# LLaVA-VL/LLaVA-Plus-Codebase

Measured on NVIDIA H100. Metric: prefill+decode tokens/s, higher is better.
Workload: dtype bf16

## Files before the change

### llava-plus-codebase_b200/csrc/decode_mega.cu

```cuda
#include <limits.h>
#include <math.h>

#include "common.cuh"
#include "kernels.h"

namespace b2 {
namespace {

constexpr int MK_CONS_WARPS = 16;
constexpr int MK_CONS = MK_CONS_WARPS * 32;
constexpr int MK_PROD_WARPS = 4;
constexpr int MK_THREADS = MK_CONS + 32 * MK_PROD_WARPS;
constexpr int MK_D = 128;
constexpr int MK_U = 4;
constexpr int MK_KT = 2048;
constexpr int MK_ROW_PAD = 64;
constexpr int MK_ROW_STRIDE = MK_KT * 2 + MK_ROW_PAD;
constexpr int MK_TILE_BYTES = 8 * MK_ROW_STRIDE;
constexpr int MK_MAXNB = 32;
constexpr int MK_MAXL = 48;
constexpr int MK_MAX_STAGES = 12;

__device__ __forceinline__ void unpack8(const uint4& u, float (&f)[8]) {
    f[0] = bf16_lo(u.x); f[1] = bf16_hi(u.x); f[2] = bf16_lo(u.y); f[3] = bf16_hi(u.y);
    f[4] = bf16_lo(u.z); f[5] = bf16_hi(u.z); f[6] = bf16_lo(u.w); f[7] = bf16_hi(u.w);
}
__device__ __forceinline__ uint4 ldcg16(const void* p) { return __ldcg(reinterpret_cast<const uint4*>(p)); }

__device__ __forceinline__ void cons_sync() { asm volatile("bar.sync 1, %0;" ::"n"(MK_CONS) : "memory"); }

__device__ __forceinline__ void grid_sync(unsigned int* counter, unsigned int target) {
    cons_sync();
    if (threadIdx.x == 0) {
        asm volatile("red.release.gpu.global.add.u32 [%0], 1;" ::"l"(counter) : "memory");
        unsigned int cur, spins = 0;
        do {
            asm volatile("ld.acquire.gpu.global.u32 %0, [%1];" : "=r"(cur) : "l"(counter) : "memory");
            if (++spins > (1u << 26)) asm volatile("trap;");
        } while ((int)(cur - target) < 0);
    }
    cons_sync();
}

__device__ __forceinline__ void bulk_g2s(void* smem_dst, const void* gsrc, uint32_t bytes, uint64_t* bar) {
    asm volatile("cp.async.bulk.shared::cluster.global.mbarrier::complete_tx::bytes [%0], [%1], %2, [%3];" ::"r"(
                     smem_u32(smem_dst)),
                 "l"(gsrc), "r"(bytes), "r"(smem_u32(bar))
                 : "memory");
}

struct GemvCtx {
    const __nv_bfloat16* W;
    int K, act;
    int u_lo, nu;
    int nb;
    int nchunk;
};
struct PhaseIO {
    const __nv_bfloat16* xin;
    const __nv_bfloat16* gamma;
    const __nv_bfloat16* residual;
    void* out;
    int ld_out, out_fp32;
};

__device__ __forceinline__ int mk_phys_row(const GemvCtx& c, int rb, int g, bool& valid) {
    if (c.act == ACT_SWIGLU) {
        const int lc = rb * 4 + (g & 3);
        valid = lc < c.nu;
        const int ch = c.u_lo + lc;
        return (ch >> 6) * 128 + (ch & 63) + ((g >> 2) ? 64 : 0);
    }
    const int lr = rb * 8 + g;
    valid = lr < c.nu;
    return c.u_lo + lr;
}

__device__ __forceinline__ int mk_rows_in_block(const GemvCtx& c, int rb) {
    if (c.act == ACT_SWIGLU) return 2 * min(4, c.nu - rb * 4);
    return min(8, c.nu - rb * 8);
// ... 79 lines not shown
#pragma unroll
                for (int e = 0; e < 8; ++e) o[e] = gf[e] * round_bf16(f[e] * rstd);
                *px = make_uint4(pack_bf16(o[0], o[1]), pack_bf16(o[2], o[3]), pack_bf16(o[4], o[5]),
                                 pack_bf16(o[6], o[7]));
            }
        }
    }
    cons_sync();
}

__device__ __forceinline__ void mk_mma(float (&c)[4], uint32_t a0, uint32_t a2, uint32_t b0, uint32_t b1) {
    asm volatile(
        "mma.sync.aligned.m16n8k16.row.col.f32.bf16.bf16.f32 {%0,%1,%2,%3}, {%4,%5,%6,%7}, {%8,%9}, {%0,%1,%2,%3};"
        : "+f"(c[0]), "+f"(c[1]), "+f"(c[2]), "+f"(c[3])
        : "r"(a0), "r"(0u), "r"(a2), "r"(0u), "r"(b0), "r"(b1));
}

template <int NB>
__device__ __forceinline__ float mk_row_value(const float* s_gpart, int rb, int b, int r) {
    float v = 0.f;
#pragma unroll
    for (int ww = 0; ww < MK_CONS_WARPS; ++ww) v += s_gpart[(((size_t)ww * MK_MAXNB + rb) * NB + b) * 8 + r];
    return v;
}

template <int NB>
__device__ __forceinline__ void mk_epilogue(const MegaParams& p, const MegaLayer* layers, int ph, const GemvCtx& c,
                                            int B, int tid, const float* s_gpart, float res_pref, bool have_res_pref) {
    const PhaseIO io = mk_phase_io(p, layers, ph);
    if (c.act == ACT_SWIGLU) {
        const int nch = c.nu;
        for (int idx = tid; idx < nch * B; idx += MK_CONS) {
            const int b = idx / nch, r = idx - b * nch;
            const int rb = r >> 2, q = r & 3;
            const float gt = mk_row_value<NB>(s_gpart, rb, b, q);
            const float up = mk_row_value<NB>(s_gpart, rb, b, q + 4);
            reinterpret_cast<__nv_bfloat16*>(io.out)[(size_t)b * io.ld_out + (size_t)c.u_lo + r] =
                __float2bfloat16_rn(gt / (1.0f + __expf(-gt)) * up);
        }
    } else {
        const int nr = c.nu;
        for (int idx = tid; idx < nr * B; idx += MK_CONS) {
            const int b = idx / nr, r = idx - b * nr;
            float y = mk_row_value<NB>(s_gpart, r >> 3, b, r & 7);
            const size_t o = (size_t)b * io.ld_out + (size_t)c.u_lo + r;
            if (io.residual != nullptr) y += have_res_pref ? res_pref : __bfloat162float(__ldcg(io.residual + o));
            if (io.out_fp32) reinterpret_cast<float*>(io.out)[o] = y;
            else reinterpret_cast<__nv_bfloat16*>(io.out)[o] = __float2bfloat16_rn(y);
        }
    }
}

__device__ __forceinline__ void mk_attention(const MegaParams& p, const MegaLayer& Lw, int tid, int lane, int warp,
                                             float (*s_part)[MK_D + 2], int* s_flag, const float* s_cos,
                                             const float* s_sin) {
    const int h = p.h, H = p.H;
    const int pairs = p.B * H;
    const int grid = gridDim.x;
    const int G = pairs <= grid ? grid / pairs : 1;
    const int hw = lane >> 4, c = lane & 15;
    const int split = pairs <= grid ? (int)blockIdx.x % G : 0;
    for (int pair = pairs <= grid ? (int)blockIdx.x / G : (int)blockIdx.x; pair < pairs;
         pair += (pairs <= grid ? pairs : grid)) {
        const int head = pair % H, b = pair / H;
        const int pos = p.cur_len[b];
        const int total = pos + 1;
        const int cchunk = (total + G - 1) / G;
        const int cb = split * cchunk;
        const int ce = min(cb + cchunk, total);
        const int wchunk = (max(ce - cb, 0) + MK_CONS_WARPS - 1) / MK_CONS_WARPS;
        const int k_begin = cb + warp * wchunk;
        const int k_end = min(k_begin + wchunk, ce);
        const __nv_bfloat16* qrow = p.qkv + (size_t)b * 3 * h + head * MK_D;
        float qreg[8], knew[8], vnew[8];
        {
            float qa[8], qb[8], ka[8], kb[8];
            unpack8(ldcg16(qrow + c * 8), qa);
            unpack8(ldcg16(qrow + (c ^ 8) * 8), qb);
            unpack8(ldcg16(qrow + h + c * 8), ka);
            unpack8(ldcg16(qrow + h + (c ^ 8) * 8), kb);
            unpack8(ldcg16(qrow + 2 * h + c * 8), vnew);
            const float sign = (c < 8) ? -1.f : 1.f;
#pragma unroll
            for (int e = 0; e < 8; ++e) {
                const int i = ((c & 7) * 8 + e);
                const float cbf = s_cos[b * 64 + i], sbf = s_sin[b * 64 + i];
                qreg[e] = round_bf16(round_bf16(qa[e] * cbf) + round_bf16(sign * qb[e] * sbf));
                knew[e] = round_bf16(round_bf16(ka[e] * cbf) + round_bf16(sign * kb[e] * sbf));
            }
        }
        const size_t cbase = ((size_t)b * H + head) * p.Smax * MK_D;
        if (pos >= k_begin && pos < k_end && hw == 0) {
            *reinterpret_cast<uint4*>(Lw.kcache + cbase + (size_t)pos * MK_D + c * 8) =
                make_uint4(pack_bf16(knew[0], knew[1]), pack_bf16(knew[2], knew[3]),
                           pack_bf16(knew[4], knew[5]), pack_bf16(knew[6], knew[7]));
            *reinterpret_cast<uint4*>(Lw.vcache + cbase + (size_t)pos * MK_D + c * 8) =
                make_uint4(pack_bf16(vnew[0], vnew[1]), pack_bf16(vnew[2], vnew[3]),
                           pack_bf16(vnew[4], vnew[5]), pack_bf16(vnew[6], vnew[7]));
        }
        float m_run = -INFINITY, l_run = 0.f, av[8];
#pragma unroll
        for (int e = 0; e < 8; ++e) av[e] = 0.f;
        const __nv_bfloat16* kb_ = Lw.kcache + cbase + c * 8;
        const __nv_bfloat16* vb_ = Lw.vcache + cbase + c * 8;
        for (int kbase = k_begin; kbase < k_end; kbase += 2 * MK_U) {
            uint4 kraw[MK_U], vraw[MK_U];
#pragma unroll
// ... 26 lines not shown
                dot += __shfl_xor_sync(0xffffffffu, dot, 1);
                if (key < k_end) {
                    const float sc = dot * p.scale_log2;
                    const float m_new = fmaxf(m_run, sc);
                    const float corr = exp2f(m_run - m_new);
                    const float pr = exp2f(sc - m_new);
                    l_run = l_run * corr + pr;
#pragma unroll
                    for (int e = 0; e < 8; ++e) av[e] = av[e] * corr + pr * vf[e];
                    m_run = m_new;
                }
            }
        }
        {
            const float m_o = __shfl_xor_sync(0xffffffffu, m_run, 16);
            const float l_o = __shfl_xor_sync(0xffffffffu, l_run, 16);
            const float m_c = fmaxf(m_run, m_o);
            const float w_s = (m_run == -INFINITY) ? 0.f : exp2f(m_run - m_c);
            const float w_o = (m_o == -INFINITY) ? 0.f : exp2f(m_o - m_c);
#pragma unroll
            for (int e = 0; e < 8; ++e) {
                const float a_o = __shfl_xor_sync(0xffffffffu, av[e], 16);
                av[e] = av[e] * w_s + a_o * w_o;
            }
            l_run = l_run * w_s + l_o * w_o;
            m_run = m_c;
        }
        if (hw == 0) {
#pragma unroll
            for (int e = 0; e < 8; ++e) s_part[warp][c * 8 + e] = av[e];
            if (c == 0) { s_part[warp][MK_D] = m_run; s_part[warp][MK_D + 1] = l_run; }
        }
        cons_sync();
        float m_cta = -INFINITY, l_cta = 0.f, o_cta = 0.f;
        if (tid < MK_D) {
#pragma unroll
            for (int i = 0; i < MK_CONS_WARPS; ++i) m_cta = fmaxf(m_cta, s_part[i][MK_D]);
#pragma unroll
            for (int i = 0; i < MK_CONS_WARPS; ++i) {
                const float ms = s_part[i][MK_D];
                const float wgt = (ms == -INFINITY) ? 0.f : exp2f(ms - m_cta);
                l_cta += s_part[i][MK_D + 1] * wgt;
                o_cta += s_part[i][tid] * wgt;
            }
        }
        if (G == 1) {
            if (tid < MK_D) p.attn[(size_t)b * h + head * MK_D + tid] = __float2bfloat16_rn(o_cta / l_cta);
        } else {
            float* part = p.attn_partial + ((size_t)pair * G + split) * (MK_D + 2);
            if (tid < MK_D) {
                part[tid] = o_cta;
                if (tid == 0) { part[MK_D] = m_cta; part[MK_D + 1] = l_cta; }
            }
            __threadfence();
            cons_sync();
            if (tid == 0) *s_flag = (atomicAdd(&p.attn_counters[pair], 1) == G - 1) ? 1 : 0;
            cons_sync();
            if (*s_flag) {
                __threadfence();
                if (tid < MK_D) {
                    const float* pb = p.attn_partial + (size_t)pair * G * (MK_D + 2);
                    float m_all = -INFINITY;
                    for (int sidx = 0; sidx < G; ++sidx) m_all = fmaxf(m_all, __ldcg(pb + (size_t)sidx * (MK_D + 2) + MK_D));
                    float l_all = 0.f, o_all = 0.f;
                    for (int sidx = 0; sidx < G; ++sidx) {
                        const float ms = __ldcg(pb + (size_t)sidx * (MK_D + 2) + MK_D);
                        const float wgt = (ms == -INFINITY) ? 0.f : exp2f(ms - m_all);
                        l_all += __ldcg(pb + (size_t)sidx * (MK_D + 2) + MK_D + 1) * wgt;
                        o_all += __ldcg(pb + (size_t)sidx * (MK_D + 2) + tid) * wgt;
                    }
                    p.attn[(size_t)b * h + head * MK_D + tid] = __float2bfloat16_rn(o_all / l_all);
                    if (tid == 0) p.attn_counters[pair] = 0;
                }
            }
        }
        cons_sync();
    }
}

struct TileCursor {
    GemvCtx c;
    int ph, rb, kc;
    uint32_t tile;
    bool valid;
};
__device__ __forceinline__ void cursor_seek(TileCursor& t, const MegaParams& p, const MegaLayer* layers, int n_phases) {
    while (t.ph < n_phases) {
        if (!mk_is_attention(p, t.ph)) {
            t.c = mk_phase_ctx(p, layers, t.ph);
            if (t.c.nb > 0) { t.rb = 0; t.kc = 0; t.valid = true; return; }
        }
        ++t.ph;
    }
    t.valid = false;
}
__device__ __forceinline__ void cursor_begin(TileCursor& t, const MegaParams& p, const MegaLayer* layers, int n_phases) {
    t.ph = 0; t.tile = 0; t.rb = 0; t.kc = 0;
    cursor_seek(t, p, layers, n_phases);
}
__device__ __forceinline__ void cursor_next(TileCursor& t, const MegaParams& p, const MegaLayer* layers, int n_phases) {
    ++t.tile;
    if (++t.kc < t.c.nchunk) return;
    t.kc = 0;
    if (++t.rb < t.c.nb) return;
    ++t.ph;
    cursor_seek(t, p, layers, n_phases);
}
template <int NB>
__global__ void __launch_bounds__(MK_THREADS, 1) decode_mega_kernel(MegaParams p, int n_stages) {
    extern __shared__ __align__(128) uint8_t mk_smem[];
    uint8_t* ring = mk_smem;
    __nv_bfloat16* xs = reinterpret_cast<__nv_bfloat16*>(ring + (size_t)n_stages * MK_TILE_BYTES);
    float* s_gpart = reinterpret_cast<float*>(reinterpret_cast<uint8_t*>(xs) + (size_t)NB * (p.h > p.I ? p.h : p.I) * 2);
    uint64_t* full_bar = reinterpret_cast<uint64_t*>(s_gpart + (size_t)MK_CONS_WARPS * MK_MAXNB * NB * 8);
    uint64_t* empty_bar = full_bar + MK_MAX_STAGES;
    __shared__ float s_red[MK_CONS_WARPS][NB];
    __shared__ float s_rstd[NB];
    __shared__ float s_av[MK_CONS_WARPS];
    __shared__ int s_ai[MK_CONS_WARPS];
    __shared__ float s_part[MK_CONS_WARPS][MK_D + 2];
    __shared__ int s_flag;
    __shared__ float s_cos[NB * 64], s_sin[NB * 64];
    __shared__ __align__(16) MegaLayer s_layers[MK_MAXL];

    const int tid = threadIdx.x, lane = tid & 31, warp = tid >> 5;
    const int B = p.B;
    const int n_phases = 5 * p.L + 1;

    {
        const uint4* src = reinterpret_cast<const uint4*>(p.layers);
        uint4* dst = reinterpret_cast<uint4*>(s_layers);
        for (int i = tid; i < p.L * (int)(sizeof(MegaLayer) / 16); i += MK_THREADS) dst[i] = src[i];
        if (tid == 0) {
            for (int s = 0; s < n_stages; ++s) {
                mbar_init(&full_bar[s], 1);
                mbar_init(&empty_bar[s], MK_CONS_WARPS);
            }
            fence_barrier_init();
        }
        __syncthreads();
    }

    if (warp >= MK_CONS_WARPS) {
        const uint32_t pw = (uint32_t)(warp - MK_CONS_WARPS);
        TileCursor cp;
        cursor_begin(cp, p, s_layers, n_phases);
        while (cp.valid) {
            if (cp.tile % (uint32_t)MK_PROD_WARPS == pw) {
                const uint32_t stage = cp.tile % (uint32_t)n_stages;
                const uint32_t parity = (cp.tile / (uint32_t)n_stages) & 1u;
                const uint32_t row_bytes = (uint32_t)min(MK_KT, cp.c.K - cp.kc * MK_KT) * 2u;
                if (lane == 0) {
                    mbar_wait(&empty_bar[stage], parity ^ 1u);
                    mbar_arrive_expect_tx(&full_bar[stage], (uint32_t)mk_rows_in_block(cp.c, cp.rb) * row_bytes);
                }
                __syncwarp();
                bool row_valid;
                const int prow = mk_phys_row(cp.c, cp.rb, lane & 7, row_valid);
                if (lane < 8 && row_valid)
                    bulk_g2s(ring + (size_t)stage * MK_TILE_BYTES + (size_t)lane * MK_ROW_STRIDE,
                             cp.c.W + (size_t)prow * cp.c.K + (size_t)cp.kc * MK_KT, row_bytes, &full_bar[stage]);
            }
            cursor_next(cp, p, s_layers, n_phases);
        }
        return;
    }

    for (int i = tid; i < B * 64; i += MK_CONS) {
        const int b = i >> 6, f = i & 63;
        const float inv_freq = exp2f(-(2.0f * f / MK_D) * log2f(p.theta));
        float sv, cv;
        sincosf((float)p.cur_len[b] * inv_freq, &sv, &cv);
        s_cos[i] = round_bf16(cv);
        s_sin[i] = round_bf16(sv);
    }
    if (blockIdx.x < B) {
        int t = p.tok[blockIdx.x];
        t = t < 0 ? 0 : (t >= p.V ? p.V - 1 : t);
        const uint4* src = reinterpret_cast<const uint4*>(p.embed + (size_t)t * p.h);
        uint4* dst = reinterpret_cast<uint4*>(p.x + (size_t)blockIdx.x * p.h);
        for (int i = tid; i < p.h / 8; i += MK_CONS) dst[i] = src[i];
    }
    __nv_bfloat16* gsm = xs + (size_t)NB * p.h;
    const bool gsm_fits = (size_t)(NB + 1) * p.h <= (size_t)NB * (p.h > p.I ? p.h : p.I);
    auto gamma_prefetch = [&](int ph) -> bool {
        if (!gsm_fits || ph >= n_phases || mk_is_attention(p, ph)) return false;
        const PhaseIO io = mk_phase_io(p, s_layers, ph);
        if (io.gamma == nullptr) return false;
        for (int i = tid; i < (p.h >> 3); i += MK_CONS)
            asm volatile("cp.async.cg.shared.global [%0], [%1], 16;" ::"r"(smem_u32(gsm + i * 8)), "l"(io.gamma + i * 8) : "memory");
        asm volatile("cp.async.commit_group;" ::: "memory");
        return true;
    };
    bool gsm_ok = gamma_prefetch(0);
    unsigned int bar_target = p.bar_base + gridDim.x;
    grid_sync(p.bar_count, bar_target);

    const bool tracing = p.trace != nullptr && blockIdx.x == 0 && tid == 0;
    const int g = lane >> 2, t4 = lane & 3;
    uint32_t tile = 0;
#pragma unroll 1
    for (int ph = 0; ph < n_phases; ++ph) {
        if (tracing) p.trace[ph * 4 + 0] = clock64();
        if (mk_is_attention(p, ph)) {
            mk_attention(p, s_layers[ph / 5], tid, lane, warp, s_part, &s_flag, s_cos, s_sin);
        } else {
            const GemvCtx c = mk_phase_ctx(p, s_layers, ph);
            const PhaseIO io = mk_phase_io(p, s_layers, ph);
            const bool have_res = io.residual != nullptr && c.nu * B <= MK_CONS;
            float res_pref = 0.f;
            if (have_res && tid < c.nu * B) {
                const int b = tid / c.nu, r = tid - b * c.nu;
                res_pref = __bfloat162float(__ldcg(io.residual + (size_t)b * io.ld_out + (size_t)c.u_lo + r));
            }
            mk_prologue<NB>(io, c.K, B, p.eps, tid, lane, warp, xs, s_red, s_rstd, gsm_ok ? gsm : nullptr);
            if (tracing) p.trace[ph * 4 + 1] = clock64();
#pragma unroll 1
            for (int rb = 0; rb < c.nb; ++rb) {
                float acc[4] = {0.f, 0.f, 0.f, 0.f}, acc2[4] = {0.f, 0.f, 0.f, 0.f};
#pragma unroll 1
                for (int kc = 0; kc < c.nchunk; ++kc, ++tile) {
                    const uint32_t stage = tile % (uint32_t)n_stages;
                    const uint32_t parity = (tile / (uint32_t)n_stages) & 1u;
                    const int nk32 = min(MK_KT, c.K - kc * MK_KT) >> 5;
                    mbar_wait(&full_bar[stage], parity);
                    const uint8_t* trow = ring + (size_t)stage * MK_TILE_BYTES + (size_t)g * MK_ROW_STRIDE + t4 * 16;
                    const __nv_bfloat16* xrow = xs + (size_t)g * c.K + (size_t)kc * MK_KT + t4 * 8;
#pragma unroll 4
                    for (int k32 = warp; k32 < nk32; k32 += MK_CONS_WARPS) {
                        const uint4 wv = *reinterpret_cast<const uint4*>(trow + k32 * 64);
                        uint4 xv = make_uint4(0, 0, 0, 0);
                        if (g < B) xv = *reinterpret_cast<const uint4*>(xrow + k32 * 32);
                        mk_mma(acc, xv.x, xv.y, wv.x, wv.y);
                        mk_mma(acc2, xv.z, xv.w, wv.z, wv.w);
                    }
                    __syncwarp();
                    if (lane == 0) mbar_arrive(&empty_bar[stage]);
                }
                if (g < NB)
                    *reinterpret_cast<float2*>(s_gpart + (((size_t)warp * MK_MAXNB + rb) * NB + g) * 8 + t4 * 2) =
                        make_float2(acc[0] + acc2[0], acc[1] + acc2[1]);
            }
            cons_sync();
            if (tracing) p.trace[ph * 4 + 2] = clock64();
            mk_epilogue<NB>(p, s_layers, ph, c, B, tid, s_gpart, res_pref, have_res);
        }
        if (tracing) p.trace[ph * 4 + 3] = clock64();
        gsm_ok = gamma_prefetch(ph + 1);
        bar_target += gridDim.x;
        grid_sync(p.bar_count, bar_target);
    }
    if (tracing) p.trace[n_phases * 4] = clock64();

    if (blockIdx.x < B) {
        const int b = blockIdx.x;
        const float* row = p.logits + (size_t)b * p.V;
        float best = -INFINITY;
        int bi = INT_MAX;
        for (int i = tid; i < p.V; i += MK_CONS) {
            const float v = __ldcg(row + i);
            if (v == v && (bi == INT_MAX || v > best)) { best = v; bi = i; }
        }
#pragma unroll
        for (int o = 16; o > 0; o >>= 1) {
            const float ov = __shfl_xor_sync(0xffffffffu, best, o);
            const int oi = __shfl_xor_sync(0xffffffffu, bi, o);
            if (ov > best || (ov == best && oi < bi)) { best = ov; bi = oi; }
        }
        if (lane == 0) { s_av[warp] = best; s_ai[warp] = bi; }
        cons_sync();
        if (warp == 0) {
            best = lane < MK_CONS_WARPS ? s_av[lane] : -INFINITY;
            bi = lane < MK_CONS_WARPS ? s_ai[lane] : INT_MAX;
#pragma unroll
            for (int o = 16; o > 0; o >>= 1) {
                const float ov = __shfl_xor_sync(0xffffffffu, best, o);
                const int oi = __shfl_xor_sync(0xffffffffu, bi, o);
                if (ov > best || (ov == best && oi < bi)) { best = ov; bi = oi; }
            }
            if (lane == 0) {
                const int tk = bi == INT_MAX ? 0 : bi;
                p.tok[b] = tk;
                p.out_tokens[(size_t)(*p.step_counter) * B + b] = tk;
                if (p.rows == nullptr || p.rows[b].active) p.cur_len[b] += 1;
                if (p.ring != nullptr) {
                    const int pub = p.sstate->pub_counter, tag0 = p.sstate->tag;
                    if (tag0 != 0) {
                        const int tag = 1 + (tag0 - 1 + pub / p.ring_cap) % 2047;
                        reinterpret_cast<volatile int32_t*>(p.ring)[(size_t)(pub % p.ring_cap) * B + b] = (tag << 20) | (tk & 0xFFFFF);
                        __threadfence_system();
                    }
                }
            }
        }
    }
    cons_sync();
    if (tid == 0) {
        __threadfence();
        if (atomicAdd(p.done_count, 1u) == gridDim.x - 1) {
            *p.done_count = 0u;
            *p.step_counter += 1;
            if (p.ring != nullptr) p.sstate->pub_counter += 1;
        }
    }
}

size_t mega_fixed_bytes(int NB, int h, int I) {
    return (size_t)NB * (h > I ? h : I) * 2 + (size_t)MK_CONS_WARPS * MK_MAXNB * NB * 8 * 4 + 2 * MK_MAX_STAGES * 8;
}
size_t mega_static_bytes(int NB) {
    return (size_t)(MK_CONS_WARPS + 1) * NB * 4 + MK_CONS_WARPS * (MK_D + 2 + 2) * 4 + NB * 512 +
           MK_MAXL * sizeof(MegaLayer) + 1024;
}
int mega_stages(int NB, int h, int I) {
    const long long avail = 227 * 1024 - (long long)mega_fixed_bytes(NB, h, I) - (long long)mega_static_bytes(NB);
    long long s = avail / MK_TILE_BYTES;
    return (int)(s > MK_MAX_STAGES ? MK_MAX_STAGES : s);
}

}

bool decode_mega_fits(int B, int h, int I) {
    if (B < 1 || B > 2) return false;
    return mega_stages(B, h, I) >= 4;
}

int decode_mega(const MegaParams& p, cudaStream_t stream) {
    B2_CHECK_ARG(p.B >= 1 && p.B <= 2, "decode_mega: batch must be 1..2");
    B2_CHECK_ARG(p.L <= MK_MAXL, "decode_mega: %d layers exceed the shared layer table (%d)", p.L, MK_MAXL);
    B2_CHECK_ARG(p.h % 256 == 0 && p.I % 256 == 0 && p.V % 8 == 0 && p.h / p.H == MK_D,
                 "decode_mega: unsupported dims h=%d I=%d V=%d H=%d", p.h, p.I, p.V, p.H);
    {
        const int grid = num_sms();
        const int nmax = p.V > 3 * p.h ? (p.V > 2 * p.I ? p.V : 2 * p.I) : (3 * p.h > 2 * p.I ? 3 * p.h : 2 * p.I);
        B2_CHECK_ARG((nmax / 8 + grid - 1) / grid + 1 <= MK_MAXNB,
                     "decode_mega: %d output rows per CTA exceed the shared-memory block table", nmax / grid);
    }
    const int NB = p.B;
    const int stages = mega_stages(NB, p.h, p.I);
    B2_CHECK_ARG(stages >= 4, "decode_mega: shared memory too small for the weight ring (B=%d h=%d I=%d)", p.B, p.h, p.I);
    const size_t smem = (size_t)stages * MK_TILE_BYTES + mega_fixed_bytes(NB, p.h, p.I);
    void* fn = NB == 1 ? (void*)decode_mega_kernel<1> : (void*)decode_mega_kernel<2>;
    static size_t attr_smem[3] = {0, 0, 0};
    if (smem > attr_smem[NB]) {
        B2_CUDA_CHECK(cudaFuncSetAttribute(fn, cudaFuncAttributeMaxDynamicSharedMemorySize, (int)smem));
        attr_smem[NB] = smem;
    }
    MegaParams pp = p;
    int n_stages = stages;
    void* args[] = {&pp, &n_stages};
    B2_CUDA_CHECK(cudaLaunchCooperativeKernel(fn, dim3(num_sms()), dim3(MK_THREADS), args, smem, stream));
    B2_LAUNCH_CHECK();
    return 0;
}

}
```

### llava-plus-codebase_b200/csrc/kernels.h

```cpp
#pragma once
#include <cuda_bf16.h>
#include <cuda_runtime.h>
#include <stdint.h>

namespace b2 {

enum { ACT_NONE = 0, ACT_QUICK_GELU = 1, ACT_GELU_ERF = 2, ACT_SWIGLU = 3, ACT_ROPE_QKV = 4 };

struct RopeQkv {
    const void* table = nullptr;
    void* kcache = nullptr;
    void* vcache = nullptr;
    int S = 0, H = 0, Smax = 0;
    const int32_t* pos0 = nullptr;
};
enum { DT_BF16 = 0, DT_F16 = 1, DT_F32 = 2 };

int num_sms();

struct GemmArgs {
    const void* A = nullptr; int lda = 0;
    const void* W = nullptr; int ldw = 0;
    const void* bias = nullptr;
    const void* residual = nullptr; int ld_res = 0;
// ... 77 lines not shown
};
int flash_attn_bf16(const FlashArgs& a, cudaStream_t stream);

int rope_table_build(void* table, int Smax, int D, float theta, cudaStream_t stream);
int rope_kv_write(void* qkv, void* kcache, void* vcache, int B, int S, int H, int D, int Smax, float theta,
                  cudaStream_t stream, const int32_t* pos0 = nullptr);

struct DecodeAttnArgs {
    const void* qkv = nullptr;
    void* kcache = nullptr; void* vcache = nullptr;
    float* kscale = nullptr; float* vscale = nullptr;
    const int32_t* cur_len = nullptr;
    void* out = nullptr;
    float* partial = nullptr;
    int32_t* counters = nullptr;
    int B = 0, H = 0, D = 128, Smax = 0, nsplit = 1;
    float theta = 10000.f, scale = 1.f;
    int R = 1;
};
int decode_attn_ctas_per_sm();
int decode_attn_bf16(const DecodeAttnArgs& a, cudaStream_t stream);
int decode_attn_mq_ctas_per_sm();
size_t decode_attn_mq_scratch_bytes(int B, int H, int nsplit);
int decode_attn_mq_bf16(const DecodeAttnArgs& a, cudaStream_t stream);
constexpr int kPrefixGroupRows = 16;
struct PrefixGroup {
    int32_t src_slot, prefix_len, n_rows;
    int32_t rows[kPrefixGroupRows];
};
int decode_attn_shared_ctas_per_sm();
size_t decode_attn_shared_scratch_bytes(int B, int H, int nsplit);
int decode_attn_shared_bf16(const DecodeAttnArgs& a, const PrefixGroup* groups, const int32_t* row_prefix, int G,
                            cudaStream_t stream);
int decode_attn_e4m3_ctas_per_sm();
int decode_attn_e4m3(const DecodeAttnArgs& a, cudaStream_t stream);
int kv_quantize_e4m3(const void* ksrc, const void* vsrc, void* k8, void* v8, float* kscale, float* vscale,
                     const int32_t* seq_lens, int B, int S, int H, int D, int Smax, cudaStream_t stream,
                     const int32_t* pos0 = nullptr, int S_src = 0);
int kv_dequantize_e4m3(const void* k8, const void* v8, const float* kscale, const float* vscale, const int32_t* pos0, void* kdst,
                       void* vdst, int B, int H, int Smax, int S_dst, cudaStream_t stream);

struct MegaLayer {
    const __nv_bfloat16 *ln1, *wqkv, *wo, *ln2, *wgu, *wd;
    __nv_bfloat16 *kcache, *vcache;
};
struct MegaParams {
    const MegaLayer* layers = nullptr;
    int L = 0, h = 0, I = 0, H = 0, V = 0, B = 0, Smax = 0, nsplit = 1;
    const __nv_bfloat16 *embed = nullptr, *final_norm = nullptr, *lm_head = nullptr;
    int32_t *tok = nullptr, *cur_len = nullptr, *out_tokens = nullptr, *step_counter = nullptr;
    __nv_bfloat16 *x = nullptr, *qkv = nullptr, *attn = nullptr, *act = nullptr;
    float* logits = nullptr;
    float* attn_partial = nullptr;
    int32_t* attn_counters = nullptr;
    unsigned int *bar_count = nullptr, *done_count = nullptr;
    unsigned int bar_base = 0;
    float eps = 1e-5f, theta = 10000.f, scale_log2 = 1.f;
    long long* trace = nullptr;
    struct SampleState* sstate = nullptr;
    int32_t* ring = nullptr;
    int ring_cap = 0;
    const struct RowState* rows = nullptr;
};
int decode_mega(const MegaParams& p, cudaStream_t stream);
bool decode_mega_fits(int B, int h, int I);

struct SampleState {
    int do_sample;
    float temperature, top_p;
    int top_k;
    unsigned long long seed;
    int tag;
    int pub_counter;
    unsigned int done;
    int per_row;
    float* out_scores;
    float* out_logits;
    int out_cap;
};
struct RowState {
    int active;
    int do_sample; float temperature, top_p; int top_k;
    unsigned long long seed;
    int index;
};
constexpr int kProcMaxEos = 8;
struct ProcRow {
    int on;
    float penalty;
    int ngram;
    int min_gen;
    int n_eos;
    int eos[kProcMaxEos];
    int prompt_len;
    int hist_len;
};
struct ProcState {
    ProcRow* rows;
    int32_t* hist;
    uint32_t* bits;
    int cap, words;
};
constexpr int kSpecMaxRows = 16;
struct SpecState {
    int K;
    int ngram;
    int max_new;
    int n_eos;
    int eos[kProcMaxEos];
// ... 86 lines not shown
```

### llava-plus-codebase_b200/csrc/model.cu

```cuda
#include <cuda_fp16.h>
#include <limits.h>
#include <stdarg.h>
#include <stdio.h>
#include <stdlib.h>
#include <string.h>
#include <time.h>

#include <array>
#include <atomic>
#include <utility>
#include <mutex>
#include <string>
#include <vector>

#include "../../include/b2llava.h"
#include "common.cuh"
#include "kernels.h"

namespace b2 {

static thread_local char g_err[1024] = {0};
unsigned long long g_launch_count = 0;

void set_error(const char* fmt, ...) {
// ... 58 lines not shown
}

using namespace b2;

struct b2_model {
    b2_model_desc d;
    int device = 0;
    std::mutex mu;
    bool finalized = false;
    int P = 0, T = 0, kpad = 0, vit_live = 0, vit_hd = 64, hd = 128;
    DevBuf patch_w, cls, pos, pre_g, pre_b;
    std::vector<VitLayer> vit;
    DevBuf p0_w, p0_b, p2_w, p2_b;
    DevBuf embed, final_norm;
    Linear head;
    std::vector<LlamaLayer> ll;
    int* err_host = nullptr;
    int* err_dev = nullptr;
    cudaEvent_t ws_event = nullptr;
    cudaStream_t ws_stream = nullptr;
    bool ws_valid = false;
    DevBuf v_col, v_patch, v_hidden, v_xn, v_qkv, v_attn, v_mlp, v_feats, p_mid, p_done;
    DevBuf x, xn, qkv, attn, act, last_idx, xlast, logits, splice_idx;
    DevBuf chunk_pos;
    DevBuf enc_pixels, enc_out;
    std::vector<cudaGraphExec_t> enc_graph;
    std::vector<char> enc_warm;
    cudaStream_t enc_stream = nullptr;
    cudaEvent_t enc_fork = nullptr, enc_join = nullptr;
    int enc_launches = 0;
    bool fp8_decode = false;
    DevBuf xq8, xscale;
    DevBuf kstage, vstage;
    bool nf4 = false;
    DevBuf nf4_scratch;
    std::atomic<int> kv_live{0};
};

struct b2_kv {
    b2_model* m = nullptr;
    int max_batch = 0, max_seq = 0;
    int dtype = B2_KV_BF16;
    int pitch = 0;
    DevBuf k, v;
    DevBuf kscale, vscale;
    DevBuf len_dev, tok, step_counter, out_tokens, attn_partial, attn_counters;
    DevBuf sk_partial, sk_counters;
    std::vector<int32_t> len_host;
    int out_capacity = 0;
    cudaGraphExec_t graph = nullptr;
    int graph_B = 0;
    int graph_launches = 0;
    unsigned int mega_bar_base = 0;
    DevBuf mega_layers, mega_sync;
    DevBuf rope_tab;
    cudaStream_t own_stream = nullptr;
    cudaEvent_t ev_fork = nullptr, ev_join = nullptr;
    int warm_B = 0;
    DevBuf sstate;
    SampleState samp_host = {};
    bool samp_valid = false;
    int32_t* ring_host = nullptr;
    int32_t* ring_dev = nullptr;
    int ring_cap = 0;
    int epoch = 0;
    int stream_B = 0, stream_tag = 0, stream_scheduled = 0;
    float* next_scores = nullptr;
    float* next_logits = nullptr;
    int next_cap = 0;
    DevBuf rows_dev;
    std::vector<RowState> rows_host;
    DevBuf beam_in, beam_ws, beam_out;
    DevBuf proc_rows, proc_hist, proc_bits;
    std::vector<char> proc_on;
    bool any_proc() const { for (char c : proc_on) if (c) return true; return false; }
    DevBuf beam_proc_rows;
    bool beam_proc_on = false;
    DevBuf spec_state, spec_logits, spec_attn;
    int* spec_mirror = nullptr;
    int spec_nsplit = 0;
    int spec_R = 0;
    int spec_max_new = 0;
    int spec_queued = 0;
    int spec_len0 = 0;
    std::array<cudaGraphExec_t, kSpecMaxRows + 1> spec_graph{};
    std::array<int, kSpecMaxRows + 1> spec_launches{};
    std::array<char, kSpecMaxRows + 1> spec_warm{};
    DevBuf share_tab, share_attn;
    int share_G = 0;
    bool counted = false;
    bool e4m3() const { return dtype == B2_KV_E4M3; }
    size_t elem_bytes() const { return e4m3() ? 1 : 2; }
    size_t layer_rows() const { return (size_t)max_batch * m->d.heads * pitch; }
    size_t layer_stride() const { return layer_rows() * m->hd; }
    char* k_layer(int l) const { return k.as<char>() + (size_t)l * layer_stride() * elem_bytes(); }
    char* v_layer(int l) const { return v.as<char>() + (size_t)l * layer_stride() * elem_bytes(); }
};

namespace {

ProcState proc_state(const b2_kv* kv) {
    ProcState p = {};
    if (kv->proc_rows.p == nullptr) return p;
    p.rows = kv->proc_rows.as<ProcRow>(); p.hist = kv->proc_hist.as<int32_t>(); p.bits = kv->proc_bits.as<uint32_t>();
    p.cap = kv->max_seq + 1; p.words = (kv->m->d.vocab + 31) / 32;
    return p;
// ... 411 lines not shown
        B2_TRY(decode_linear(m, kv, p, L.d, lw.wd, m->act.p, I, nullptr, true, m->x.p, h, 0, B, h, I, ACT_NONE, st));
    }
    B2_TRY(decode_linear(m, kv, plan.head, m->head, m->head.w.p, m->x.p, h, m->final_norm.p, false, m->logits.p, V, 1, B, V, h,
                         ACT_NONE, st));
    B2_TRY(sample_publish(m->logits.as<float>(), V, B, kv->sstate.as<SampleState>(), kv->rows_dev.as<RowState>(), kv->tok.as<int32_t>(),
                          kv->out_tokens.as<int32_t>(), kv->step_counter.as<int32_t>(), kv->len_dev.as<int32_t>(),
                          kv->ring_dev, kv->ring_cap, SP_SELECT | SP_WRITE_OUT | SP_BUMP, 0, proc_state(kv), nullptr, st));
    return 0;
}

int fork_stream(b2_kv* kv, cudaStream_t st, cudaStream_t* run) {
    if (st != nullptr && st != cudaStreamLegacy) { *run = st; return 0; }
    if (kv->own_stream == nullptr) {
        B2_CUDA_CHECK(cudaStreamCreateWithFlags(&kv->own_stream, cudaStreamNonBlocking));
        B2_CUDA_CHECK(cudaEventCreateWithFlags(&kv->ev_fork, cudaEventDisableTiming));
        B2_CUDA_CHECK(cudaEventCreateWithFlags(&kv->ev_join, cudaEventDisableTiming));
    }
    B2_CUDA_CHECK(cudaEventRecord(kv->ev_fork, st));
    B2_CUDA_CHECK(cudaStreamWaitEvent(kv->own_stream, kv->ev_fork, 0));
    *run = kv->own_stream;
    return 0;
}
int join_stream(b2_kv* kv, cudaStream_t st, cudaStream_t run) {
    if (run == st) return 0;
    B2_CUDA_CHECK(cudaEventRecord(kv->ev_join, run));
    B2_CUDA_CHECK(cudaStreamWaitEvent(st, kv->ev_join, 0));
    return 0;
}

bool use_mega(const b2_model* m, const b2_kv* kv, int B) {
    if (kv->e4m3()) return false;
    if (m->nf4) return false;
    if (!decode_mega_fits(B, m->d.hidden, m->d.inter) || m->d.layers > 48) return false;
    static int flag = -1;
    if (flag < 0) {
        const char* e = getenv("B2_DECODE_MEGA");
        flag = (e != nullptr && e[0] == '0') ? 0 : 1;
    }
    return flag == 1;
}

int decode_step_mega(b2_model* m, b2_kv* kv, int B, cudaStream_t st) {
    const b2_model_desc& d = m->d;
    MegaParams p;
    p.layers = kv->mega_layers.as<MegaLayer>();
    p.L = d.layers; p.h = d.hidden; p.I = d.inter; p.H = d.heads; p.V = d.vocab; p.B = B; p.Smax = kv->pitch;
    int ns = (num_sms() * 16) / (B * d.heads);
    p.nsplit = ns < 1 ? 1 : (ns > 64 ? 64 : ns);
    p.embed = m->embed.as<bf16>(); p.final_norm = m->final_norm.as<bf16>(); p.lm_head = m->head.w.as<bf16>();
    p.tok = kv->tok.as<int32_t>(); p.cur_len = kv->len_dev.as<int32_t>();
    p.out_tokens = kv->out_tokens.as<int32_t>(); p.step_counter = kv->step_counter.as<int32_t>();
    p.x = m->x.as<bf16>(); p.qkv = m->qkv.as<bf16>(); p.attn = m->attn.as<bf16>(); p.act = m->act.as<bf16>();
    p.logits = m->logits.as<float>();
    p.attn_partial = kv->attn_partial.as<float>(); p.attn_counters = kv->attn_counters.as<int32_t>();
    unsigned int* sync = kv->mega_sync.as<unsigned int>();
    p.bar_count = sync; p.done_count = sync + 2;
    p.bar_base = kv->mega_bar_base;
    kv->mega_bar_base += (unsigned int)(5 * d.layers + 2) * (unsigned int)num_sms();
    p.eps = d.rms_eps; p.theta = d.rope_theta;
    p.scale_log2 = (1.0f / sqrtf((float)m->hd)) * 1.4426950408889634f;
    const bool sampling = kv->samp_host.do_sample != 0 || kv->samp_host.per_row != 0 || kv->any_proc();
    if (!sampling && kv->samp_host.tag != 0) { p.sstate = kv->sstate.as<SampleState>(); p.ring = kv->ring_dev; p.ring_cap = kv->ring_cap; }
    if (kv->samp_host.per_row) p.rows = kv->rows_dev.as<RowState>();
    static int trace_mode = -1;
    if (trace_mode < 0) { const char* e = getenv("B2_MEGA_TRACE"); trace_mode = (e && e[0] != 0) ? 1 : 0; }
    if (trace_mode == 1) {
        static int steps_seen = 0;
        if (++steps_seen == 40) {
            const int n = (5 * d.layers + 2) * 4;
            DevBuf tb;
            B2_TRY(tb.alloc((size_t)n * 8));
            cudaMemset(tb.p, 0, (size_t)n * 8);
            p.trace = tb.as<long long>();
            int r = decode_mega(p, st);
            cudaStreamSynchronize(st);
            std::vector<long long> host(n);
            cudaMemcpy(host.data(), tb.p, (size_t)n * 8, cudaMemcpyDeviceToHost);
            FILE* f = fopen(getenv("B2_MEGA_TRACE"), "w");
            if (f) {
                for (int ph = 0; ph <= 5 * d.layers; ++ph)
                    fprintf(f, "%d %lld %lld %lld %lld %lld\n", ph, host[ph * 4], host[ph * 4 + 1], host[ph * 4 + 2],
                            host[ph * 4 + 3], host[(ph + 1) * 4]);
                fclose(f);
            }
            tb.free();
            return r;
        }
    }
    B2_TRY(decode_mega(p, st));
    if (!sampling && p.ring != nullptr && kv->samp_host.out_cap > 0)
        B2_TRY(publish_rows(m->logits.as<float>(), d.vocab, B, kv->sstate.as<SampleState>(), st));
    if (sampling)
        B2_TRY(sample_publish(m->logits.as<float>(), d.vocab, B, kv->sstate.as<SampleState>(), kv->rows_dev.as<RowState>(), kv->tok.as<int32_t>(),
                              kv->out_tokens.as<int32_t>(), kv->step_counter.as<int32_t>(), kv->len_dev.as<int32_t>(),
                              kv->ring_dev, kv->ring_cap, SP_SELECT | SP_WRITE_OUT, -1, proc_state(kv), nullptr, st));
    return 0;
}

static void share_arm(b2_kv* kv, int G) {
    if (kv->share_G == G) return;
    if (kv->graph) { cudaGraphExecDestroy(kv->graph); kv->graph = nullptr; kv->graph_B = 0; }
    kv->warm_B = 0;
    kv->share_G = G;
}
int decode_step_run(b2_model* m, b2_kv* kv, int B, cudaStream_t st) {
    if (use_mega(m, kv, B)) return decode_step_mega(m, kv, B, st);
    if (kv->warm_B != B) {
        if (kv->graph) { cudaGraphExecDestroy(kv->graph); kv->graph = nullptr; kv->graph_B = 0; }
        B2_TRY(decode_step_launch(m, kv, B, st));
        kv->warm_B = B;
        return 0;
    }
    if (kv->graph == nullptr || kv->graph_B != B) {
        if (kv->graph) { cudaGraphExecDestroy(kv->graph); kv->graph = nullptr; }
        B2_TRY(capture_graph(st, &kv->graph, &kv->graph_launches, [&] { return decode_step_launch(m, kv, B, st); }));
        kv->graph_B = B;
    }
    B2_CUDA_CHECK(cudaGraphLaunch(kv->graph, st));
    g_launch_count += (unsigned long long)kv->graph_launches;
    return 0;
}

int32_t* spec_rows(b2_kv* kv) { return reinterpret_cast<int32_t*>(kv->spec_state.as<char>() + offsetof(SpecState, rows)); }

int rows_forward(b2_model* m, b2_kv* kv, int slot, int R, cudaStream_t st) {
    const b2_model_desc& d = m->d;
    const int h = d.hidden, I = d.inter, H = d.heads, V = d.vocab;
    const DecodePlan plan = decode_plan(m, kv, R);
    const DecodePath p = plan.layer;
    const int32_t* len = kv->len_dev.as<int32_t>() + slot;
    const size_t slot_off = (size_t)slot * H * kv->pitch * m->hd * kv->elem_bytes();
    const size_t attn_partial = decode_attn_mq_scratch_bytes(1, H, kv->spec_nsplit) - (size_t)H * sizeof(int32_t);
    B2_TRY(embed_tokens(spec_rows(kv), m->embed.p, m->x.p, R, h, V, m->err_dev, st));
    for (int l = 0; l < d.layers; ++l) {
        LlamaLayer& L = m->ll[l];
        LayerW lw = {};
        if (p != GEMV_NF4) B2_TRY(layer_weights(m, l, &lw, st));
        B2_TRY(decode_linear(m, kv, p, L.qkv, lw.wqkv, m->x.p, h, L.ln1.p, false, m->qkv.p, 3 * h, 0, R, 3 * h, h, ACT_NONE, st));
        B2_TRY(rope_kv_write(m->qkv.p, kv->k_layer(l) + slot_off, kv->v_layer(l) + slot_off, 1, R, H, m->hd, kv->pitch,
                             d.rope_theta, st, len));
        DecodeAttnArgs da;
        da.qkv = m->qkv.p;
// ... 1922 lines not shown
```

Measured before the change: 705.7.

## Replace post-attention grid barrier with head-count wait and merge split-K partials in o_proj prologue

Attention CTAs no longer elect a last-arriver to merge the split-KV partials. Each CTA bumps a global head counter, and consumers spin on that counter instead of a full grid barrier after attention. Every CTA then merges the partials for the full hidden vector directly into shared memory as the o_proj prologue. This removes the atomic and threadfence handshake plus one grid barrier per layer, but every CTA now redundantly reads all partials. Per-block tracing is also reworked to record stall and globaltimer timestamps.

```diff
diff --git a/llava-plus-codebase_b200/csrc/decode_mega.cu b/llava-plus-codebase_b200/csrc/decode_mega.cu
--- a/llava-plus-codebase_b200/csrc/decode_mega.cu
+++ b/llava-plus-codebase_b200/csrc/decode_mega.cu
@@ -26,6 +26,11 @@
     f[4] = bf16_lo(u.z); f[5] = bf16_hi(u.z); f[6] = bf16_lo(u.w); f[7] = bf16_hi(u.w);
 }
 __device__ __forceinline__ uint4 ldcg16(const void* p) { return __ldcg(reinterpret_cast<const uint4*>(p)); }
+__device__ __forceinline__ long long globaltimer_ns() {
+    unsigned long long t;
+    asm volatile("mov.u64 %0, %%globaltimer;" : "=l"(t));
+    return (long long)t;
+}
 
 __device__ __forceinline__ void cons_sync() { asm volatile("bar.sync 1, %0;" ::"n"(MK_CONS) : "memory"); }
 
@@ -211,7 +216,7 @@
 }
 
 __device__ __forceinline__ void mk_attention(const MegaParams& p, const MegaLayer& Lw, int tid, int lane, int warp,
-                                             float (*s_part)[MK_D + 2], int* s_flag, const float* s_cos,
+                                             float (*s_part)[MK_D + 2], const float* s_cos,
                                              const float* s_sin) {
     const int h = p.h, H = p.H;
     const int pairs = p.B * H;
@@ -344,30 +349,58 @@
                 part[tid] = o_cta;
                 if (tid == 0) { part[MK_D] = m_cta; part[MK_D + 1] = l_cta; }
             }
-            __threadfence();
-            cons_sync();
-            if (tid == 0) *s_flag = (atomicAdd(&p.attn_counters[pair], 1) == G - 1) ? 1 : 0;
-            cons_sync();
-            if (*s_flag) {
-                __threadfence();
-                if (tid < MK_D) {
-                    const float* pb = p.attn_partial + (size_t)pair * G * (MK_D + 2);
-                    float m_all = -INFINITY;
-                    for (int sidx = 0; sidx < G; ++sidx) m_all = fmaxf(m_all, __ldcg(pb + (size_t)sidx * (MK_D + 2) + MK_D));
-                    float l_all = 0.f, o_all = 0.f;
-                    for (int sidx = 0; sidx < G; ++sidx) {
-                        const float ms = __ldcg(pb + (size_t)sidx * (MK_D + 2) + MK_D);
-                        const float wgt = (ms == -INFINITY) ? 0.f : exp2f(ms - m_all);
-                        l_all += __ldcg(pb + (size_t)sidx * (MK_D + 2) + MK_D + 1) * wgt;
-                        o_all += __ldcg(pb + (size_t)sidx * (MK_D + 2) + tid) * wgt;
+        }
+        cons_sync();
+        if (tid == 0)
+            asm volatile("red.release.gpu.global.add.u32 [%0], 1;" ::"l"(p.head_count) : "memory");
+    }
+}
+
+template <int NB>
+__device__ __forceinline__ void mk_attn_merge(const MegaParams& p, int G, int B, int tid, __nv_bfloat16* xs) {
+    const int K = p.h, nvec = K >> 3;
+    for (int i = tid; i < nvec; i += MK_CONS) {
+        const int head = (i * 8) / MK_D, d = (i * 8) % MK_D;
+#pragma unroll
+        for (int b = 0; b < NB; ++b) {
+            uint4 u = make_uint4(0, 0, 0, 0);
+            if (b < B) {
+                const float* pb = p.attn_partial + (size_t)(b * p.H + head) * G * (MK_D + 2);
+                float m_all = -INFINITY;
+                for (int sidx = 0; sidx < G; ++sidx) m_all = fmaxf(m_all, __ldcg(pb + (size_t)sidx * (MK_D + 2) + MK_D));
+                float l_all = 0.f, o[8];
+#pragma unroll
+                for (int e = 0; e < 8; ++e) o[e] = 0.f;
+                for (int sidx = 0; sidx < G; ++sidx) {
+                    const float* ps = pb + (size_t)sidx * (MK_D + 2);
+                    const float ms = __ldcg(ps + MK_D);
+                    const float wgt = (ms == -INFINITY) ? 0.f : exp2f(ms - m_all);
+                    l_all += __ldcg(ps + MK_D + 1) * wgt;
+#pragma unroll
+                    for (int e = 0; e < 8; e += 2) {
+                        const float2 v = __ldcg(reinterpret_cast<const float2*>(ps + d + e));
+                        o[e] += v.x * wgt;
+                        o[e + 1] += v.y * wgt;
                     }
-                    p.attn[(size_t)b * h + head * MK_D + tid] = __float2bfloat16_rn(o_all / l_all);
-                    if (tid == 0) p.attn_counters[pair] = 0;
                 }
-            }
-        }
-        cons_sync();
-    }
+                u = make_uint4(pack_bf16(o[0] / l_all, o[1] / l_all), pack_bf16(o[2] / l_all, o[3] / l_all),
+                               pack_bf16(o[4] / l_all, o[5] / l_all), pack_bf16(o[6] / l_all, o[7] / l_all));
+            }
+            *reinterpret_cast<uint4*>(xs + (size_t)b * K + i * 8) = u;
+        }
+    }
+    cons_sync();
+}
+
+__device__ __forceinline__ void mk_heads_wait(const unsigned int* counter, unsigned int target) {
+    if (threadIdx.x == 0) {
+        unsigned int cur, spins = 0;
+        do {
+            asm volatile("ld.acquire.gpu.global.u32 %0, [%1];" : "=r"(cur) : "l"(counter) : "memory");
+            if (++spins > (1u << 26)) asm volatile("trap;");
+        } while ((int)(cur - target) < 0);
+    }
+    cons_sync();
 }
 
 struct TileCursor {
@@ -411,13 +444,13 @@
     __shared__ float s_av[MK_CONS_WARPS];
     __shared__ int s_ai[MK_CONS_WARPS];
     __shared__ float s_part[MK_CONS_WARPS][MK_D + 2];
-    __shared__ int s_flag;
     __shared__ float s_cos[NB * 64], s_sin[NB * 64];
     __shared__ __align__(16) MegaLayer s_layers[MK_MAXL];
 
     const int tid = threadIdx.x, lane = tid & 31, warp = tid >> 5;
     const int B = p.B;
     const int n_phases = 5 * p.L + 1;
+    long long* const tr = p.trace != nullptr ? p.trace + (size_t)blockIdx.x * (n_phases + 1) * 4 : nullptr;
 
     {
         const uint4* src = reinterpret_cast<const uint4*>(p.layers);
@@ -437,13 +470,16 @@
         const uint32_t pw = (uint32_t)(warp - MK_CONS_WARPS);
         TileCursor cp;
         cursor_begin(cp, p, s_layers, n_phases);
+        long long stall = 0;
         while (cp.valid) {
             if (cp.tile % (uint32_t)MK_PROD_WARPS == pw) {
                 const uint32_t stage = cp.tile % (uint32_t)n_stages;
                 const uint32_t parity = (cp.tile / (uint32_t)n_stages) & 1u;
                 const uint32_t row_bytes = (uint32_t)min(MK_KT, cp.c.K - cp.kc * MK_KT) * 2u;
                 if (lane == 0) {
+                    const long long t0 = tr != nullptr ? clock64() : 0;
                     mbar_wait(&empty_bar[stage], parity ^ 1u);
+                    if (tr != nullptr) stall += clock64() - t0;
                     mbar_arrive_expect_tx(&full_bar[stage], (uint32_t)mk_rows_in_block(cp.c, cp.rb) * row_bytes);
                 }
                 __syncwarp();
@@ -453,11 +489,18 @@
                     bulk_g2s(ring + (size_t)stage * MK_TILE_BYTES + (size_t)lane * MK_ROW_STRIDE,
                              cp.c.W + (size_t)prow * cp.c.K + (size_t)cp.kc * MK_KT, row_bytes, &full_bar[stage]);
             }
+            const int ph = cp.ph;
             cursor_next(cp, p, s_layers, n_phases);
+            if (tr != nullptr && lane == 0 && (cp.ph != ph || !cp.valid)) {
+                atomicMax(reinterpret_cast<unsigned long long*>(tr + ph * 4 + 2), (unsigned long long)stall);
+                stall = 0;
+            }
         }
         return;
     }
 
+    const bool tracing = tr != nullptr && tid == 0;
+    if (tracing) { tr[n_phases * 4 + 0] = clock64(); tr[n_phases * 4 + 1] = globaltimer_ns(); }
     for (int i = tid; i < B * 64; i += MK_CONS) {
         const int b = i >> 6, f = i & 63;
         const float inv_freq = exp2f(-(2.0f * f / MK_D) * log2f(p.theta));
@@ -488,14 +531,14 @@
     unsigned int bar_target = p.bar_base + gridDim.x;
     grid_sync(p.bar_count, bar_target);
 
-    const bool tracing = p.trace != nullptr && blockIdx.x == 0 && tid == 0;
     const int g = lane >> 2, t4 = lane & 3;
+    unsigned int head_target = p.head_base;
+    const int attn_G = B * p.H <= (int)gridDim.x ? (int)gridDim.x / (B * p.H) : 1;
     uint32_t tile = 0;
 #pragma unroll 1
     for (int ph = 0; ph < n_phases; ++ph) {
-        if (tracing) p.trace[ph * 4 + 0] = clock64();
         if (mk_is_attention(p, ph)) {
-            mk_attention(p, s_layers[ph / 5], tid, lane, warp, s_part, &s_flag, s_cos, s_sin);
+            mk_attention(p, s_layers[ph / 5], tid, lane, warp, s_part, s_cos, s_sin);
         } else {
             const GemvCtx c = mk_phase_ctx(p, s_layers, ph);
             const PhaseIO io = mk_phase_io(p, s_layers, ph);
@@ -505,8 +548,8 @@
                 const int b = tid / c.nu, r = tid - b * c.nu;
                 res_pref = __bfloat162float(__ldcg(io.residual + (size_t)b * io.ld_out + (size_t)c.u_lo + r));
             }
-            mk_prologue<NB>(io, c.K, B, p.eps, tid, lane, warp, xs, s_red, s_rstd, gsm_ok ? gsm : nullptr);
-            if (tracing) p.trace[ph * 4 + 1] = clock64();
+            if (ph % 5 == 2 && ph < 5 * p.L && attn_G > 1) mk_attn_merge<NB>(p, attn_G, B, tid, xs);
+            else mk_prologue<NB>(io, c.K, B, p.eps, tid, lane, warp, xs, s_red, s_rstd, gsm_ok ? gsm : nullptr);
 #pragma unroll 1
             for (int rb = 0; rb < c.nb; ++rb) {
                 float acc[4] = {0.f, 0.f, 0.f, 0.f}, acc2[4] = {0.f, 0.f, 0.f, 0.f};
@@ -534,15 +577,19 @@
                         make_float2(acc[0] + acc2[0], acc[1] + acc2[1]);
             }
             cons_sync();
-            if (tracing) p.trace[ph * 4 + 2] = clock64();
             mk_epilogue<NB>(p, s_layers, ph, c, B, tid, s_gpart, res_pref, have_res);
         }
-        if (tracing) p.trace[ph * 4 + 3] = clock64();
+        if (tracing) tr[ph * 4 + 0] = clock64();
         gsm_ok = gamma_prefetch(ph + 1);
-        bar_target += gridDim.x;
-        grid_sync(p.bar_count, bar_target);
-    }
-    if (tracing) p.trace[n_phases * 4] = clock64();
+        if (mk_is_attention(p, ph)) {
+            head_target += (unsigned int)(B * p.H * attn_G);
+            mk_heads_wait(p.head_count, head_target);
+        } else {
+            bar_target += gridDim.x;
+            grid_sync(p.bar_count, bar_target);
+        }
+        if (tracing) { tr[ph * 4 + 1] = clock64(); tr[ph * 4 + 3] = globaltimer_ns(); }
+    }
 
     if (blockIdx.x < B) {
         const int b = blockIdx.x;
@@ -595,6 +642,7 @@
             if (p.ring != nullptr) p.sstate->pub_counter += 1;
         }
     }
+    if (tracing) { tr[n_phases * 4 + 2] = clock64(); tr[n_phases * 4 + 3] = globaltimer_ns(); }
 }
 
 size_t mega_fixed_bytes(int NB, int h, int I) {
diff --git a/llava-plus-codebase_b200/csrc/kernels.h b/llava-plus-codebase_b200/csrc/kernels.h
--- a/llava-plus-codebase_b200/csrc/kernels.h
+++ b/llava-plus-codebase_b200/csrc/kernels.h
@@ -153,9 +153,10 @@
     __nv_bfloat16 *x = nullptr, *qkv = nullptr, *attn = nullptr, *act = nullptr;
     float* logits = nullptr;
     float* attn_partial = nullptr;
-    int32_t* attn_counters = nullptr;
     unsigned int *bar_count = nullptr, *done_count = nullptr;
     unsigned int bar_base = 0;
+    unsigned int* head_count = nullptr;
+    unsigned int head_base = 0;
     float eps = 1e-5f, theta = 10000.f, scale_log2 = 1.f;
     long long* trace = nullptr;
     struct SampleState* sstate = nullptr;
diff --git a/llava-plus-codebase_b200/csrc/model.cu b/llava-plus-codebase_b200/csrc/model.cu
--- a/llava-plus-codebase_b200/csrc/model.cu
+++ b/llava-plus-codebase_b200/csrc/model.cu
@@ -134,6 +134,7 @@
     int graph_B = 0;
     int graph_launches = 0;
     unsigned int mega_bar_base = 0;
+    unsigned int mega_head_base = 0;
     DevBuf mega_layers, mega_sync;
     DevBuf rope_tab;
     cudaStream_t own_stream = nullptr;
@@ -651,11 +652,15 @@
     p.out_tokens = kv->out_tokens.as<int32_t>(); p.step_counter = kv->step_counter.as<int32_t>();
     p.x = m->x.as<bf16>(); p.qkv = m->qkv.as<bf16>(); p.attn = m->attn.as<bf16>(); p.act = m->act.as<bf16>();
     p.logits = m->logits.as<float>();
-    p.attn_partial = kv->attn_partial.as<float>(); p.attn_counters = kv->attn_counters.as<int32_t>();
+    p.attn_partial = kv->attn_partial.as<float>();
     unsigned int* sync = kv->mega_sync.as<unsigned int>();
     p.bar_count = sync; p.done_count = sync + 2;
+    p.head_count = sync + 8;
     p.bar_base = kv->mega_bar_base;
-    kv->mega_bar_base += (unsigned int)(5 * d.layers + 2) * (unsigned int)num_sms();
+    kv->mega_bar_base += (unsigned int)(4 * d.layers + 2) * (unsigned int)num_sms();
+    p.head_base = kv->mega_head_base;
+    const int pairs = B * d.heads, attn_G = pairs <= num_sms() ? num_sms() / pairs : 1;
+    kv->mega_head_base += (unsigned int)(d.layers * pairs * attn_G);
     p.eps = d.rms_eps; p.theta = d.rope_theta;
     p.scale_log2 = (1.0f / sqrtf((float)m->hd)) * 1.4426950408889634f;
     const bool sampling = kv->samp_host.do_sample != 0 || kv->samp_host.per_row != 0 || kv->any_proc();
@@ -663,30 +668,28 @@
     if (kv->samp_host.per_row) p.rows = kv->rows_dev.as<RowState>();
     static int trace_mode = -1;
     if (trace_mode < 0) { const char* e = getenv("B2_MEGA_TRACE"); trace_mode = (e && e[0] != 0) ? 1 : 0; }
-    if (trace_mode == 1) {
-        static int steps_seen = 0;
-        if (++steps_seen == 40) {
-            const int n = (5 * d.layers + 2) * 4;
-            DevBuf tb;
-            B2_TRY(tb.alloc((size_t)n * 8));
-            cudaMemset(tb.p, 0, (size_t)n * 8);
-            p.trace = tb.as<long long>();
-            int r = decode_mega(p, st);
-            cudaStreamSynchronize(st);
-            std::vector<long long> host(n);
-            cudaMemcpy(host.data(), tb.p, (size_t)n * 8, cudaMemcpyDeviceToHost);
-            FILE* f = fopen(getenv("B2_MEGA_TRACE"), "w");
-            if (f) {
-                for (int ph = 0; ph <= 5 * d.layers; ++ph)
-                    fprintf(f, "%d %lld %lld %lld %lld %lld\n", ph, host[ph * 4], host[ph * 4 + 1], host[ph * 4 + 2],
-                            host[ph * 4 + 3], host[(ph + 1) * 4]);
-                fclose(f);
-            }
-            tb.free();
-            return r;
-        }
+    static int steps_seen = 0;
+    static DevBuf tb;
+    const size_t trace_launch = (size_t)num_sms() * (5 * d.layers + 2) * 4;
+    if (trace_mode == 1 && ++steps_seen >= 40 && steps_seen <= 41) {
+        if (steps_seen == 40) {
+            B2_TRY(tb.alloc(2 * trace_launch * 8));
+            cudaMemsetAsync(tb.p, 0, 2 * trace_launch * 8, st);
+        }
+        p.trace = tb.as<long long>() + (steps_seen - 40) * trace_launch;
     }
     B2_TRY(decode_mega(p, st));
+    if (p.trace != nullptr && steps_seen == 41) {
+        cudaStreamSynchronize(st);
+        std::vector<long long> host(4 + 2 * trace_launch);
+        host[0] = 2; host[1] = num_sms(); host[2] = 5 * d.layers + 2; host[3] = 4;
+        cudaMemcpy(host.data() + 4, tb.p, 2 * trace_launch * 8, cudaMemcpyDeviceToHost);
+        if (FILE* f = fopen(getenv("B2_MEGA_TRACE"), "wb")) {
+            fwrite(host.data(), 8, host.size(), f);
+            fclose(f);
+        }
+        tb.free();
+    }
     if (!sampling && p.ring != nullptr && kv->samp_host.out_cap > 0)
         B2_TRY(publish_rows(m->logits.as<float>(), d.vocab, B, kv->sstate.as<SampleState>(), st));
     if (sampling)
```

After: 695.2, median of 6. 0.985x the previous value.
